# mindazhao/PWStableNet

Measured on AMD Instinct MI355X. Metric: stabilized frames/sec at 256x256 (netG fp32 + grid_sample), whole job, higher is better.
Workload: dtype f32

## Files before the change

### pwstablenet_amd/csrc/conv_mfma.hip

```cpp
#include "conv_common.h"

namespace pws {

template <int KS_, int STRIDE_, int PAD_, int SUBPIX_, int TH_, int TW_, int TN_, int CK_, int WM_, int WN_, int MT_,
          int NT_, bool NCHW_ = false>
struct ConvCfg {
    static constexpr int KS = KS_, STRIDE = STRIDE_, PAD = PAD_, TH = TH_, TW = TW_, TN = TN_, CK = CK_;
    static constexpr int SUBPIX = SUBPIX_;
    static constexpr bool CONVT = SUBPIX_ != 0, NCHW = NCHW_;
    static constexpr int WM = WM_, WN = WN_, MT = MT_, NT = NT_;
    static constexpr int THREADS = 64 * WM * WN;
    static constexpr int BM = TH * TW * TN, BN = 32 * NT * WN;
    static_assert(BM == 32 * MT * WM, "tile pixels must equal the M extent of the wave grid");
    static constexpr int IH = (TH - 1) * STRIDE + KS, IW = (TW - 1) * STRIDE + KS;
    static constexpr int PIX = TN * IH * IW;
    static constexpr int CKP = CK + 1;
    static constexpr int TAPS = KS * KS;
    static constexpr int LDS_IN = (PIX * CKP + 3) / 4 * 4;
    static constexpr int LDS_W = TAPS * CK * BN;
    static constexpr int LDS_BYTES = (LDS_IN + LDS_W) * 4;
    static constexpr int C4 = CK / 4;
    static constexpr int ITEMS_IN = (PIX * C4 + THREADS - 1) / THREADS;
    static constexpr int ITEMS_W = (TAPS * CK * (BN / 4) + THREADS - 1) / THREADS;
    static constexpr int ITEMS_NCHW = (PIX * CK + THREADS - 1) / THREADS;
// ... 47 lines not shown
        const int item = tid + it * C::THREADS;
        const int row = item / (C::BN / 4), q = item % (C::BN / 4);
        const int tap = row / C::CK, c = row % C::CK;
        const bool ok = item < C::TAPS * C::CK * (C::BN / 4) && (co0 + q * 4) < p.cout;
        w_off[it] = ok ? (tap * p.cin_pad + c) * p.cout + co0 + q * 4 : 0;
        w_mask |= ok ? (1u << it) : 0u;
    }
    const float *w_cls = p.w + (size_t)cls * C::TAPS * p.cin_pad * p.cout;
    float4 r_in[C::NCHW ? 1 : C::ITEMS_IN];
    float4 r_w[C::ITEMS_W];
    float r_nchw[C::NCHW ? C::ITEMS_NCHW : 1];

    auto load_chunk = [&](int s, int c0, int wrow) {
        if constexpr (C::NCHW) {
            const int Creal = p.src_c[0];
            const size_t sstride = p.src_ld[0] ? (size_t)p.src_ld[0] : (size_t)Creal * p.H * p.W;
#pragma unroll
            for (int it = 0; it < C::ITEMS_NCHW; ++it) {
                const int item = tid + it * C::THREADS;
                const int c = item / C::PIX, pix = item % C::PIX;
                const int lx = pix % C::IW, ly = (pix / C::IW) % C::IH, tn = pix / (C::IW * C::IH);
                const int n = n0 + tn, iy = iy0 + ly, ix = ix0 + lx;
                const bool ok = item < C::PIX * C::CK && (c0 + c) < Creal && n < p.N && iy >= 0 && iy < p.H && ix >= 0 &&
                                ix < p.W;
                const size_t off = ok ? (size_t)n * sstride + ((size_t)(c0 + c) * p.H + iy) * p.W + ix : 0;
                const float v = p.src_ptr[0][off];
                r_nchw[it] = ok ? v : 0.f;
            }
        } else {
            const float *sp = p.src_ptr[s] + c0;
            const size_t ld = p.src_ld[s];
#pragma unroll
            for (int it = 0; it < C::ITEMS_IN; ++it)
                r_in[it] = *reinterpret_cast<const float4 *>(sp + (size_t)g_pix[it] * ld + g_c4[it]);
        }
        const float *wp = w_cls + (size_t)wrow * p.cout;
#pragma unroll
        for (int it = 0; it < C::ITEMS_W; ++it) r_w[it] = *reinterpret_cast<const float4 *>(wp + w_off[it]);
    };
    auto store_chunk = [&]() {
        if constexpr (C::NCHW) {
#pragma unroll
            for (int it = 0; it < C::ITEMS_NCHW; ++it) {
                const int item = tid + it * C::THREADS;
                const int c = item / C::PIX, pix = item % C::PIX;
                if (item < C::PIX * C::CK) lds_in[pix * C::CKP + c] = r_nchw[it];
            }
        } else {
#pragma unroll
            for (int it = 0; it < C::ITEMS_IN; ++it) {
                if (l_off[it] >= 0) {
                    const bool ok = (ok_mask >> it) & 1u;
                    float *d = lds_in + l_off[it];
                    d[0] = ok ? r_in[it].x : 0.f, d[1] = ok ? r_in[it].y : 0.f, d[2] = ok ? r_in[it].z : 0.f,
                    d[3] = ok ? r_in[it].w : 0.f;
                }
            }
        }
#pragma unroll
        for (int it = 0; it < C::ITEMS_W; ++it) {
            const int item = tid + it * C::THREADS;
            if (item < C::TAPS * C::CK * (C::BN / 4)) {
                const bool ok = (w_mask >> it) & 1u;
                *reinterpret_cast<float4 *>(lds_w + item * 4) =
                    ok ? r_w[it] : make_float4(0.f, 0.f, 0.f, 0.f);
            }
        }
    };

    f32x16 acc[C::MT][C::NT];
#pragma unroll
    for (int mt = 0; mt < C::MT; ++mt)
#pragma unroll
        for (int nt = 0; nt < C::NT; ++nt)
#pragma unroll
            for (int r = 0; r < 16; ++r) acc[mt][nt][r] = 0.f;

    int a_base[C::MT];
#pragma unroll
    for (int mt = 0; mt < C::MT; ++mt) {
        const int m = (wm * C::MT + mt) * 32 + l31;
        const int tx = m % C::TW, ty = (m / C::TW) % C::TH, tn = m / (C::TW * C::TH);
        a_base[mt] = ((tn * C::IH + ty * C::STRIDE) * C::IW + tx * C::STRIDE) * C::CKP + hi;
    }
    const int b_base = hi * C::BN + wn * C::NT * 32 + l31;

    int total_chunks = 0;
    if constexpr (C::NCHW) {
        total_chunks = p.cin_pad / C::CK;
    } else {
        for (int s = 0; s < p.nsrc; ++s) total_chunks += p.src_c[s] / C::CK;
    }
    const int ch_begin = split * p.chunks_per_split;
    const int ch_end = min(total_chunks, ch_begin + p.chunks_per_split);
    int s = 0, c0 = ch_begin * C::CK, wrow = ch_begin * C::CK;
    if constexpr (!C::NCHW) {
        while (s < p.nsrc - 1 && c0 >= p.src_c[s]) c0 -= p.src_c[s], ++s;
    }
    if (ch_begin < ch_end) load_chunk(s, c0, wrow);
    for (int ch = ch_begin; ch < ch_end; ++ch) {
        __syncthreads();
        store_chunk();
        __syncthreads();
        c0 += C::CK, wrow += C::CK;
        if (!C::NCHW && c0 >= p.src_c[s]) ++s, c0 = 0;
        if (ch + 1 < ch_end) load_chunk(s, c0, wrow);

#pragma unroll
        for (int tap = 0; tap < C::TAPS; ++tap) {
            if (C::SUBPIX == 2 && ((!py && tap / C::KS) || (!px && tap % C::KS))) continue;
            const int toff = ((tap / C::KS) * C::IW + (tap % C::KS)) * C::CKP;
#pragma unroll
            for (int kk = 0; kk < C::CK / 2; ++kk) {
                float a[C::MT], b[C::NT];
#pragma unroll
                for (int mt = 0; mt < C::MT; ++mt) a[mt] = lds_in[a_base[mt] + toff + 2 * kk];
#pragma unroll
                for (int nt = 0; nt < C::NT; ++nt) b[nt] = lds_w[b_base + (tap * C::CK + 2 * kk) * C::BN + nt * 32];
#pragma unroll
                for (int mt = 0; mt < C::MT; ++mt)
#pragma unroll
                    for (int nt = 0; nt < C::NT; ++nt)
                        acc[mt][nt] = __builtin_amdgcn_mfma_f32_32x32x2f32(a[mt], b[nt], acc[mt][nt], 0, 0, 0);
            }
        }
    }

    const bool partial = p.ksplit > 1;
    float *part = p.out + (size_t)split * p.split_stride;
#pragma unroll
    for (int nt = 0; nt < C::NT; ++nt) {
        const int co = co0 + (wn * C::NT + nt) * 32 + l31;
        const bool co_ok = co < p.cout;
#pragma unroll
        for (int mt = 0; mt < C::MT; ++mt) {
#pragma unroll
            for (int r = 0; r < 16; ++r) {
                const int m = (wm * C::MT + mt) * 32 + (r & 3) + 8 * (r >> 2) + 4 * hi;
                const int tx = m % C::TW, ty = (m / C::TW) % C::TH, tn = m / (C::TW * C::TH);
                const int n = n0 + tn, y = y0 + ty, x = x0 + tx;
                const int oy = C::CONVT ? 2 * y + py : y, ox = C::CONVT ? 2 * x + px : x;
                if (co_ok && n < p.N && y < p.LH && x < p.LW && oy < p.OH && ox < p.OW) {
                    const size_t pix = (size_t)(n * p.OH + oy) * p.OW + ox;
                    if (partial)
                        part[pix * p.cout + co] = acc[mt][nt][r];
                    else
                        epi_store(p, pix, co, acc[mt][nt][r]);
                }
            }
        }
    }
}

__global__ void __launch_bounds__(256) splitk_reduce_kernel(const ConvKParams p, const float *__restrict__ partial,
                                                            size_t total4) {
    const size_t i = (size_t)blockIdx.x * 256 + threadIdx.x;
    if (i >= total4) return;
    float4 a = reinterpret_cast<const float4 *>(partial)[i];
    for (int s = 1; s < p.ksplit; ++s) {
        const float4 b = reinterpret_cast<const float4 *>(partial + (size_t)s * p.split_stride)[i];
        a.x += b.x, a.y += b.y, a.z += b.z, a.w += b.w;
    }
    const size_t pix = (i * 4) / p.cout;
    const int co = (int)((i * 4) % p.cout);
    if (p.io_bf16) {
        epi_store_pair16(p, pix, co, a.x, a.y), epi_store_pair16(p, pix, co + 2, a.z, a.w);
        return;
    }
    epi_store(p, pix, co, a.x), epi_store(p, pix, co + 1, a.y), epi_store(p, pix, co + 2, a.z), epi_store(p, pix, co + 3, a.w);
}

int launch_splitk_reduce(const ConvKParams &kp, const float *partial, size_t total4, hipStream_t st) {
    hipLaunchKernelGGL(splitk_reduce_kernel, dim3((unsigned)((total4 + 255) / 256)), dim3(256), 0, st, kp, partial, total4);
    return check_launch("splitk_reduce_kernel");
}

template <class C>
static int run_cfg(const ConvKParams &kp, const ConvChoice &c, hipStream_t st) { return launch_planned<&conv_mfma_kernel<C>>(kp, c, st, "conv_mfma_kernel"); }

template <class C, int KID>
static constexpr TileChoice choice() {
    return TileChoice{C::TH, C::TW, C::TN, C::CK, C::BN, KID, {{C::THREADS, C::LDS_BYTES}, {C::THREADS, C::LDS_BYTES}}, &run_cfg<C>};
}

using K3S1_T256 = ConvCfg<3, 1, 1, 0, 16, 16, 1, 16, 4, 1, 2, 2>;
using K3S1_T128 = ConvCfg<3, 1, 1, 0, 8, 16, 1, 16, 4, 1, 1, 2>;
using K3S1_T64 = ConvCfg<3, 1, 1, 0, 8, 8, 1, 16, 2, 2, 1, 1>;
using K3S1_T64N4 = ConvCfg<3, 1, 1, 0, 4, 4, 4, 16, 2, 2, 1, 1>;
using K3S1_T64N16 = ConvCfg<3, 1, 1, 0, 2, 2, 16, 16, 2, 2, 1, 1>;
using K3S2_T256 = ConvCfg<3, 2, 1, 0, 16, 16, 1, 8, 4, 1, 2, 2>;
using K3S2_T128 = ConvCfg<3, 2, 1, 0, 8, 16, 1, 16, 4, 1, 1, 2>;
using K3S2_T64 = ConvCfg<3, 2, 1, 0, 8, 8, 1, 16, 2, 2, 1, 1>;
using K3S2_T64N4 = ConvCfg<3, 2, 1, 0, 4, 4, 4, 16, 2, 2, 1, 1>;
using K3S2_T64N16 = ConvCfg<3, 2, 1, 0, 2, 2, 16, 16, 2, 2, 1, 1>;
using K5S1_T256 = ConvCfg<5, 1, 2, 0, 16, 16, 1, 8, 4, 1, 2, 2>;
using K5S1_T256_NCHW = ConvCfg<5, 1, 2, 0, 16, 16, 1, 8, 4, 1, 2, 2, true>;
using CT4_T256 = ConvCfg<2, 1, 0, 1, 16, 16, 1, 16, 4, 1, 2, 2>;
using CT4_T128 = ConvCfg<2, 1, 0, 1, 8, 16, 1, 16, 4, 1, 1, 2>;
using CT4_T64 = ConvCfg<2, 1, 0, 1, 8, 8, 1, 16, 2, 2, 1, 1>;
using CT4_T64N4 = ConvCfg<2, 1, 0, 1, 4, 4, 4, 16, 2, 2, 1, 1>;
using CT4_T64N16 = ConvCfg<2, 1, 0, 1, 2, 2, 16, 16, 2, 2, 1, 1>;

using K4S2_T256 = ConvCfg<4, 2, 1, 0, 16, 16, 1, 8, 4, 1, 2, 2>;
using K4S2_T128 = ConvCfg<4, 2, 1, 0, 8, 16, 1, 8, 4, 1, 1, 2>;
using K4S2_T64 = ConvCfg<4, 2, 1, 0, 8, 8, 1, 8, 2, 2, 1, 1>;
using K4S2_T64N4 = ConvCfg<4, 2, 1, 0, 4, 4, 4, 8, 2, 2, 1, 1>;
using K4S2_T64N16 = ConvCfg<4, 2, 1, 0, 2, 2, 16, 8, 2, 2, 1, 1>;
using SP3_T256 = ConvCfg<2, 1, 0, 2, 16, 16, 1, 16, 4, 1, 2, 2>;
using SP3_T128 = ConvCfg<2, 1, 0, 2, 8, 16, 1, 16, 4, 1, 1, 2>;
using SP3_T64 = ConvCfg<2, 1, 0, 2, 8, 8, 1, 16, 2, 2, 1, 1>;
using SP3_T64N4 = ConvCfg<2, 1, 0, 2, 4, 4, 4, 16, 2, 2, 1, 1>;
using SP3_T64N16 = ConvCfg<2, 1, 0, 2, 2, 2, 16, 16, 2, 2, 1, 1>;

static const TileChoice kK3S1[] = {choice<K3S1_T256, KID_CONV_K3S1_BIG>(), choice<K3S1_T128, KID_CONV_K3S1_BIG>(),
                                   choice<K3S1_T64, KID_CONV_K3S1_SMALL>(), choice<K3S1_T64N4, KID_CONV_K3S1_SMALL>(),
                                   choice<K3S1_T64N16, KID_CONV_K3S1_SMALL>()};
static const TileChoice kK3S2[] = {choice<K3S2_T256, KID_CONV_K3S2_BIG>(), choice<K3S2_T128, KID_CONV_K3S2_BIG>(),
                                   choice<K3S2_T64, KID_CONV_K3S2_SMALL>(), choice<K3S2_T64N4, KID_CONV_K3S2_SMALL>(),
                                   choice<K3S2_T64N16, KID_CONV_K3S2_SMALL>()};
static const TileChoice kCT4[] = {choice<CT4_T256, KID_CONVT4_BIG>(), choice<CT4_T128, KID_CONVT4_BIG>(),
                                  choice<CT4_T64, KID_CONVT4_SMALL>(), choice<CT4_T64N4, KID_CONVT4_SMALL>(),
                                  choice<CT4_T64N16, KID_CONVT4_SMALL>()};
static const TileChoice kK4S2[] = {choice<K4S2_T256, KID_DGRAD_K4S2>(), choice<K4S2_T128, KID_DGRAD_K4S2>(),
                                   choice<K4S2_T64, KID_DGRAD_K4S2>(), choice<K4S2_T64N4, KID_DGRAD_K4S2>(),
                                   choice<K4S2_T64N16, KID_DGRAD_K4S2>()};
static const TileChoice kSP3[] = {choice<SP3_T256, KID_DGRAD_SP3>(), choice<SP3_T128, KID_DGRAD_SP3>(),
                                  choice<SP3_T64, KID_DGRAD_SP3>(), choice<SP3_T64N4, KID_DGRAD_SP3>(),
                                  choice<SP3_T64N16, KID_DGRAD_SP3>()};
static const TileChoice kK5[] = {choice<K5S1_T256, KID_CONV_K5S1>()};
static const TileChoice kK5N[] = {choice<K5S1_T256_NCHW, KID_CONV_K5S1>()};

bool conv_mfma(int kind, bool dgrad, bool nchw, ConvKParams &kp, int cin_total, float *final_out, float *ws, size_t ws_floats, const ProfInfo &pi,
               const ConvCtx &cx, int *status) {
    const bool s1 = kind == PWS_CONV_K3S1 || kind == PWS_CONVT_K3S1, k5 = kind == PWS_CONV_K5S1;
    const TileChoice *cands = s1 ? kK3S1 : k5 ? (nchw ? kK5N : kK5) : kind == PWS_CONV_K3S2 ? (dgrad ? kSP3 : kK3S2) : (dgrad ? kK4S2 : kCT4);
    const int ncand = k5 ? 1 : 5;
    ConvChoice c;
    const TileChoice *t = plan_tiles(cands, ncand, kp, cin_total, final_out, ws, ws_floats, kFillBlocks, 0, &c);
    return conv_accept(cx, c, pi, status, [&] { return run_tiles(*t, c, kp, final_out, ws, cx.stream); });
}

}
```

### pwstablenet_amd/csrc/head.hip

```cpp
#include <type_traits>

#include "common.h"

namespace pws {

__device__ __forceinline__ float lrelu(float v) { return v > 0.f ? v : 0.2f * v; }

constexpr int TH_NB = 8;

__global__ void __launch_bounds__(64) theta_hidden_kernel(const float *__restrict__ x, int n, int k1, int hidden, int kchunk,
                                                          const float *__restrict__ w_flat, float *__restrict__ partial) {
    extern __shared__ float sx[];
    const int lane = threadIdx.x;
    const int j = blockIdx.x * 64 + lane;
    const int slice = blockIdx.y;
    const int k0 = slice * kchunk, kn = min(kchunk, k1 - k0);
    for (int n0 = blockIdx.z * TH_NB; n0 < n; n0 += gridDim.z * TH_NB) {
        const int nb = min(TH_NB, n - n0);
        __syncthreads();
        for (int i = lane; i < nb * kn; i += 64) sx[(i / kn) * kchunk + i % kn] = x[(size_t)(n0 + i / kn) * k1 + k0 + i % kn];
        __syncthreads();
        float acc[TH_NB];
#pragma unroll
        for (int s = 0; s < TH_NB; ++s) acc[s] = 0.f;
        if (j < hidden) {
            for (int kb = 0; kb < kn; kb += 8) {
                float wv[8];
#pragma unroll
                for (int u = 0; u < 8; ++u) wv[u] = w_flat[(size_t)(k0 + (kb + u < kn ? kb + u : kb)) * hidden + j];
#pragma unroll
                for (int u = 0; u < 8; ++u) {
                    if (kb + u < kn) {
#pragma unroll
                        for (int s = 0; s < TH_NB; ++s) acc[s] = fmaf(s < nb ? sx[s * kchunk + kb + u] : 0.f, wv[u], acc[s]);
                    }
                }
            }
#pragma unroll
            for (int s = 0; s < TH_NB; ++s)
                if (s < nb) partial[((size_t)slice * n + n0 + s) * hidden + j] = acc[s];
        }
    }
}

__global__ void __launch_bounds__(256) theta_final_kernel(const float *__restrict__ partial, int nslices, int n, int hidden,
                                                          const float *__restrict__ b_flat, const float *__restrict__ w_lin,
                                                          const float *__restrict__ b_lin, float *__restrict__ theta,
                                                          float *__restrict__ h_saved) {
    extern __shared__ float sh[];
    const int s = blockIdx.x, tid = threadIdx.x;
    for (int j = tid; j < hidden; j += 256) {
        float acc = b_flat ? b_flat[j] : 0.f;
        for (int sl = 0; sl < nslices; ++sl) acc += partial[((size_t)sl * n + s) * hidden + j];
        sh[j] = lrelu(acc);
        if (h_saved) h_saved[(size_t)s * hidden + j] = sh[j];
    }
    __syncthreads();
    const int wv = tid >> 6, lane = tid & 63;
    for (int o = wv; o < 6; o += 4) {
        float acc = 0.f;
        for (int j = lane; j < hidden; j += 64) acc = fmaf(sh[j], w_lin[(size_t)j * 6 + o], acc);
#pragma unroll
        for (int off = 32; off > 0; off >>= 1) acc += __shfl_down(acc, off, 64);
        if (lane == 0) theta[(size_t)s * 6 + o] = lrelu(acc + (b_lin ? b_lin[o] : 0.f));
    }
}

constexpr int FH_T = 16, FH_I = FH_T + 2, FH_CH = 16, FH_LDP = FH_CH + 4;

template <bool IO16>
__global__ void __launch_bounds__(256) field_head_kernel(const float *__restrict__ x, int ld, int N, int H, int W, int C,
                                                         const float *__restrict__ w_out, const float *__restrict__ b_out,
                                                         const float *__restrict__ theta, int ac, float *__restrict__ resid,
                                                         float *__restrict__ grid, int tiles_x, int tiles_y, unsigned ntiles, int raw) {
    __shared__ float s_in[FH_I * FH_I * FH_LDP];
    const int tid = threadIdx.x;
    const unsigned tile = xcd_remap(blockIdx.x, ntiles);
    const int tx_i = tile % tiles_x, ty_i = (tile / tiles_x) % tiles_y, n = tile / (tiles_x * tiles_y);
    const int x0 = tx_i * FH_T, y0 = ty_i * FH_T;
    const int tx = tid & 15, ty = tid >> 4;
    const int ch = C < FH_CH ? C : FH_CH;
    const int c4n = ch / 4;
    float acc0 = b_out ? b_out[0] : 0.f, acc1 = b_out ? b_out[1] : 0.f;
    constexpr int NITEM = (FH_I * FH_I * (FH_CH / 4) + 255) / 256;
    float4 pre[NITEM];
    auto fetch = [&](int c0) {
#pragma unroll
        for (int it = 0; it < NITEM; ++it) {
            const int item = tid + it * 256;
            const int pix = item / c4n, c4 = item % c4n;
            const int iy = y0 - 1 + pix / FH_I, ix = x0 - 1 + pix % FH_I;
            const bool ok = item < FH_I * FH_I * c4n && iy >= 0 && iy < H && ix >= 0 && ix < W;
            const float4 v = ld4<IO16>(x, ok ? ((size_t)(n * H + iy) * W + ix) * ld + c0 + c4 * 4 : 0);
            pre[it] = ok ? v : make_float4(0.f, 0.f, 0.f, 0.f);
        }
    };
    fetch(0);
    for (int c0 = 0; c0 < C; c0 += ch) {
        __syncthreads();
#pragma unroll
        for (int it = 0; it < NITEM; ++it) {
            const int item = tid + it * 256;
            if (item < FH_I * FH_I * c4n) *reinterpret_cast<float4 *>(s_in + (item / c4n) * FH_LDP + (item % c4n) * 4) = pre[it];
        }
        __syncthreads();
        if (c0 + ch < C) fetch(c0 + ch);
#pragma unroll
        for (int tap = 0; tap < 9; ++tap) {
            const float *ip = s_in + ((ty + tap / 3) * FH_I + tx + tap % 3) * FH_LDP;
            const float *wp = w_out + ((size_t)tap * C + c0) * 2;
            for (int c4 = 0; c4 < c4n; ++c4) {
                const float4 v = *reinterpret_cast<const float4 *>(ip + c4 * 4);
                const float *wq = wp + c4 * 8;
                acc0 = fmaf(v.x, wq[0], acc0), acc1 = fmaf(v.x, wq[1], acc1);
                acc0 = fmaf(v.y, wq[2], acc0), acc1 = fmaf(v.y, wq[3], acc1);
                acc0 = fmaf(v.z, wq[4], acc0), acc1 = fmaf(v.z, wq[5], acc1);
                acc0 = fmaf(v.w, wq[6], acc0), acc1 = fmaf(v.w, wq[7], acc1);
            }
        }
    }
    const int y = y0 + ty, xq = x0 + tx;
    if (y < H && xq < W && raw) {
        *reinterpret_cast<float2 *>(resid + (((size_t)n * H + y) * W + xq) * 2) = make_float2(acc0, acc1);
    } else if (y < H && xq < W) {
        const float r0 = tanhf(tanhf(acc0)), r1 = tanhf(tanhf(acc1));
        const size_t p = ((size_t)n * H + y) * W + xq;
        if (resid) *reinterpret_cast<float2 *>(resid + p * 2) = make_float2(r0, r1);
        if (grid) {
            float a0 = 0.f, a1 = 0.f;
            if (theta) {
                const float *t = theta + (size_t)n * 6;
                const float bx = ac ? (W > 1 ? (2.f * xq) / (float)(W - 1) - 1.f : 0.f) : (2.f * xq + 1.f) / (float)W - 1.f;
                const float by = ac ? (H > 1 ? (2.f * y) / (float)(H - 1) - 1.f : 0.f) : (2.f * y + 1.f) / (float)H - 1.f;
                a0 = t[0] * bx + t[1] * by + t[2];
                a1 = t[3] * bx + t[4] * by + t[5];
            }
            *reinterpret_cast<float2 *>(grid + p * 2) = make_float2(r0 + a0, r1 + a1);
        }
    }
}


__global__ void __launch_bounds__(256) field_head16_mfma_kernel(const __bf16 *__restrict__ x, int ld, int N, int H, int W,
                                                                const float *__restrict__ w_out, const float *__restrict__ b_out,
                                                                const float *__restrict__ theta, int ac, float *__restrict__ resid,
                                                                float *__restrict__ grid, int tiles_x, int tiles_y, unsigned ntiles, int raw) {
    constexpr int C = 64, NPIX = FH_I * FH_I, YP = 18;
    __shared__ float ys[NPIX * YP];
    typedef float f32x16 __attribute__((ext_vector_type(16)));
    const int tid = threadIdx.x, lane = tid & 63, wv = tid >> 6, l31 = lane & 31, hi = lane >> 5;
    bf16x8 bh[4], bl[4], bl2[4];
    {
        const int tap = l31 >> 1, o = l31 & 1;
#pragma unroll
        for (int ks = 0; ks < 4; ++ks)
#pragma unroll
            for (int i = 0; i < 8; ++i) {
                const float w = l31 < 18 ? w_out[((size_t)tap * C + ks * 16 + hi * 8 + i) * 2 + o] : 0.f;
                const __bf16 h = (__bf16)w;
                const float r1 = w - (float)h;
                const __bf16 m = (__bf16)r1;
                bh[ks][i] = h, bl[ks][i] = m, bl2[ks][i] = (__bf16)(r1 - (float)m);
            }
    }
    constexpr int MT = (NPIX + 31) / 32;
    constexpr int MTW = (MT + 3) / 4;
    bf16x8 a[MTW][4];
    auto load_tile = [&](unsigned t) {
        const unsigned tile = xcd_remap(t, ntiles);
        const int tx_i = tile % tiles_x, ty_i = (tile / tiles_x) % tiles_y, n = tile / (tiles_x * tiles_y);
        const int x0 = tx_i * FH_T, y0 = ty_i * FH_T;
#pragma unroll
        for (int i = 0; i < MTW; ++i) {
            const int q = (wv + 4 * i) * 32 + l31;
            const int iy = y0 - 1 + q / FH_I, ix = x0 - 1 + q % FH_I;
            const bool ok = q < NPIX && iy >= 0 && iy < H && ix >= 0 && ix < W;
            const __bf16 *px = x + (ok ? ((size_t)(n * H + iy) * W + ix) * ld + hi * 8 : 0);
#pragma unroll
            for (int ks = 0; ks < 4; ++ks) {
                const u32x4 v = *reinterpret_cast<const u32x4 *>(px + ks * 16);
                a[i][ks] = __builtin_bit_cast(bf16x8, ok ? v : (u32x4){0u, 0u, 0u, 0u});
            }
        }
    };
    unsigned t = blockIdx.x;
    if (t >= ntiles) return;
    load_tile(t);
    const float bias0 = b_out ? b_out[0] : 0.f, bias1 = b_out ? b_out[1] : 0.f;
    for (;;) {
        const unsigned tile = xcd_remap(t, ntiles);
        const int tx_i = tile % tiles_x, ty_i = (tile / tiles_x) % tiles_y, n = tile / (tiles_x * tiles_y);
        const int x0 = tx_i * FH_T, y0 = ty_i * FH_T;
#pragma unroll
        for (int i = 0; i < MTW; ++i) {
            const int mt = wv + 4 * i;
            if (mt >= MT) break;
            f32x16 acc;
#pragma unroll
            for (int r = 0; r < 16; ++r) acc[r] = 0.f;
#pragma unroll
            for (int ks = 0; ks < 4; ++ks) {
                acc = __builtin_amdgcn_mfma_f32_32x32x16_bf16(a[i][ks], bh[ks], acc, 0, 0, 0);
                acc = __builtin_amdgcn_mfma_f32_32x32x16_bf16(a[i][ks], bl[ks], acc, 0, 0, 0);
                acc = __builtin_amdgcn_mfma_f32_32x32x16_bf16(a[i][ks], bl2[ks], acc, 0, 0, 0);
            }
            if (l31 < 18) {
#pragma unroll
                for (int r = 0; r < 16; ++r) {
                    const int qq = mt * 32 + (r & 3) + 8 * (r >> 2) + 4 * hi;
                    if (qq < NPIX) ys[qq * YP + l31] = acc[r];
                }
            }
        }
        const unsigned tn = t + gridDim.x;
// ... 158 lines not shown
        }
        __syncthreads();
#pragma unroll
        for (int h2 = 0; h2 < 2; ++h2) {
            const int idx = tid + h2 * 256;
            const int ty = idx >> 5, tx = idx & 31;
            float acc0 = bias0, acc1 = bias1;
#pragma unroll
            for (int tap = 0; tap < 9; ++tap) {
                const float2 v = *reinterpret_cast<const float2 *>(ysr + (h2 * 8 * F2_IW + (tap / 3) * F2_IW + tap % 3) * F2_YP + tap * 2);
                acc0 += v.x, acc1 += v.y;
            }
            const int y = T.y0 + ty, xq = T.x0 + tx;
            if (y < H && xq < W && raw) {
                *reinterpret_cast<float2 *>(resid + (((size_t)T.n * H + y) * W + xq) * 2) = make_float2(acc0, acc1);
            } else if (y < H && xq < W) {
                const float r0 = tanhf(tanhf(acc0)), r1 = tanhf(tanhf(acc1));
                const size_t pp = ((size_t)T.n * H + y) * W + xq;
                if (resid) *reinterpret_cast<float2 *>(resid + pp * 2) = make_float2(r0, r1);
                if (grid) {
                    float a0 = 0.f, a1 = 0.f;
                    if (theta) {
                        const float *th = theta + (size_t)T.n * 6;
                        const float bx = (ac && W <= 1) ? 0.f : (float)(2 * xq + 1 - ac) / (float)(W - ac) - 1.f;
                        const float by = (ac && H <= 1) ? 0.f : (float)(2 * y + 1 - ac) / (float)(H - ac) - 1.f;
                        a0 = th[0] * bx + th[1] * by + th[2];
                        a1 = th[3] * bx + th[4] * by + th[5];
                    }
                    *reinterpret_cast<float2 *>(grid + pp * 2) = make_float2(r0 + a0, r1 + a1);
                }
            }
        }
        __syncthreads();
    };
    auto advance = [&]() {
        T = TN, t = tn, tn += gridDim.x;
        more = tn < ntiles;
        if (more) TN = decode(tn);
    };
    for (;;) {
        do_tile(std::integral_constant<int, 0>{});
        if (!more) break;
        advance();
        do_tile(std::integral_constant<int, F2_BPW % NSET>{});
        if (!more) break;
        advance();
        if constexpr (NSET == 3) {
            do_tile(std::integral_constant<int, (2 * F2_BPW) % NSET>{});
            if (!more) break;
            advance();
        }
    }
}

__global__ void __launch_bounds__(256) field_head32_mfma_kernel(const float *__restrict__ x, int ld, int N, int H, int W,
                                                                const float *__restrict__ w_out, const float *__restrict__ b_out,
                                                                const float *__restrict__ theta, int ac, float *__restrict__ resid,
                                                                float *__restrict__ grid, int tiles_x, int tiles_y, unsigned ntiles, int raw) {
    constexpr int C = 64, NPIX = FH_I * FH_I, YP = 18;
    __shared__ float ys[NPIX * YP];
    typedef float f32x16 __attribute__((ext_vector_type(16)));
    const int tid = threadIdx.x, lane = tid & 63, wv = tid >> 6, l31 = lane & 31, hi = lane >> 5;
    float bw[32];
    {
        const int tap = l31 >> 1, o = l31 & 1;
#pragma unroll
        for (int j = 0; j < 32; ++j) bw[j] = l31 < 18 ? w_out[((size_t)tap * C + hi * 32 + j) * 2 + o] : 0.f;
    }
    constexpr int MT = (NPIX + 31) / 32, MTW = (MT + 3) / 4;
    f32x4 a[MTW][8];
    auto load_tile = [&](unsigned t) {
        const unsigned tile = xcd_remap(t, ntiles);
        const int tx_i = tile % tiles_x, ty_i = (tile / tiles_x) % tiles_y, n = tile / (tiles_x * tiles_y);
        const int x0 = tx_i * FH_T, y0 = ty_i * FH_T;
#pragma unroll
        for (int i = 0; i < MTW; ++i) {
            const int q = (wv + 4 * i) * 32 + l31;
            const int iy = y0 - 1 + q / FH_I, ix = x0 - 1 + q % FH_I;
            const bool ok = q < NPIX && iy >= 0 && iy < H && ix >= 0 && ix < W;
            const float *px = x + (ok ? ((size_t)(n * H + iy) * W + ix) * ld + hi * 32 : 0);
#pragma unroll
            for (int k4 = 0; k4 < 8; ++k4) {
                const f32x4 v = *reinterpret_cast<const f32x4 *>(px + k4 * 4);
                a[i][k4] = ok ? v : (f32x4){0.f, 0.f, 0.f, 0.f};
            }
        }
    };
    unsigned t = blockIdx.x;
    if (t >= ntiles) return;
    load_tile(t);
    const float bias0 = b_out ? b_out[0] : 0.f, bias1 = b_out ? b_out[1] : 0.f;
    for (;;) {
        const unsigned tile = xcd_remap(t, ntiles);
        const int tx_i = tile % tiles_x, ty_i = (tile / tiles_x) % tiles_y, n = tile / (tiles_x * tiles_y);
        const int x0 = tx_i * FH_T, y0 = ty_i * FH_T;
#pragma unroll
        for (int i = 0; i < MTW; ++i) {
            const int mt = wv + 4 * i;
            if (mt >= MT) break;
            f32x16 acc;
#pragma unroll
            for (int r = 0; r < 16; ++r) acc[r] = 0.f;
#pragma unroll
            for (int j = 0; j < 32; ++j) acc = __builtin_amdgcn_mfma_f32_32x32x2f32(a[i][j >> 2][j & 3], bw[j], acc, 0, 0, 0);
            if (l31 < 18) {
#pragma unroll
                for (int r = 0; r < 16; ++r) {
                    const int qq = mt * 32 + (r & 3) + 8 * (r >> 2) + 4 * hi;
                    if (qq < NPIX) ys[qq * YP + l31] = acc[r];
                }
            }
        }
        const unsigned tn = t + gridDim.x;
        const bool more = tn < ntiles;
        if (more) load_tile(tn);
        __syncthreads();
        const int tx = tid & 15, ty = tid >> 4;
        float acc0 = bias0, acc1 = bias1;
#pragma unroll
        for (int tap = 0; tap < 9; ++tap) {
            const float2 v = *reinterpret_cast<const float2 *>(ys + ((ty + tap / 3) * FH_I + tx + tap % 3) * YP + tap * 2);
            acc0 += v.x, acc1 += v.y;
        }
        const int y = y0 + ty, xq = x0 + tx;
        if (y < H && xq < W && raw) {
            *reinterpret_cast<float2 *>(resid + (((size_t)n * H + y) * W + xq) * 2) = make_float2(acc0, acc1);
        } else if (y < H && xq < W) {
            const float r0 = tanhf(tanhf(acc0)), r1 = tanhf(tanhf(acc1));
            const size_t p = ((size_t)n * H + y) * W + xq;
            if (resid) *reinterpret_cast<float2 *>(resid + p * 2) = make_float2(r0, r1);
            if (grid) {
                float a0 = 0.f, a1 = 0.f;
                if (theta) {
                    const float *th = theta + (size_t)n * 6;
                    const float bx = ac ? (W > 1 ? (2.f * xq) / (float)(W - 1) - 1.f : 0.f) : (2.f * xq + 1.f) / (float)W - 1.f;
                    const float by = ac ? (H > 1 ? (2.f * y) / (float)(H - 1) - 1.f : 0.f) : (2.f * y + 1.f) / (float)H - 1.f;
                    a0 = th[0] * bx + th[1] * by + th[2];
                    a1 = th[3] * bx + th[4] * by + th[5];
                }
                *reinterpret_cast<float2 *>(grid + p * 2) = make_float2(r0 + a0, r1 + a1);
            }
        }
        if (!more) break;
        __syncthreads();
        t = tn;
    }
}

__global__ void __launch_bounds__(256) theta_sum_kernel(const float *__restrict__ partial, int nslices, int n, int hidden,
                                                        const float *__restrict__ b_flat, float *__restrict__ z1) {
    const size_t e = (size_t)blockIdx.x * 256 + threadIdx.x;
    if (e >= (size_t)n * hidden) return;
    const int j = (int)(e % hidden);
    float acc = b_flat ? b_flat[j] : 0.f;
    for (int sl = 0; sl < nslices; ++sl) acc += partial[(size_t)sl * n * hidden + e];
    z1[e] = acc;
}
__global__ void __launch_bounds__(256) theta_z2_kernel(const float *__restrict__ h, int n, int hidden, const float *__restrict__ w_lin,
                                                       const float *__restrict__ b_lin, float *__restrict__ z2) {
    const int wave = (int)(((size_t)blockIdx.x * 256 + threadIdx.x) >> 6), lane = threadIdx.x & 63;
    if (wave >= n * 6) return;
    const int s = wave / 6, o = wave % 6;
    float acc = 0.f;
    for (int j = lane; j < hidden; j += 64) acc = fmaf(h[(size_t)s * hidden + j], w_lin[(size_t)j * 6 + o], acc);
#pragma unroll
    for (int off = 32; off > 0; off >>= 1) acc += __shfl_down(acc, off, 64);
    if (lane == 0) z2[(size_t)s * 6 + o] = acc + (b_lin ? b_lin[o] : 0.f);
}
__global__ void __launch_bounds__(256) field_bn_finish_kernel(const float *__restrict__ yhat, const float *__restrict__ theta, int H, int W,
                                                              size_t total, int ac, float *__restrict__ resid, float *__restrict__ grid) {
    const size_t p = (size_t)blockIdx.x * 256 + threadIdx.x;
    if (p >= total) return;
    const float2 v = *reinterpret_cast<const float2 *>(yhat + p * 2);
    const float r0 = tanhf(tanhf(v.x)), r1 = tanhf(tanhf(v.y));
    if (resid) *reinterpret_cast<float2 *>(resid + p * 2) = make_float2(r0, r1);
    if (grid) {
        const int xq = (int)(p % W), y = (int)((p / W) % H);
        const size_t n = p / ((size_t)W * H);
        float a0 = 0.f, a1 = 0.f;
        if (theta) {
            const float *t = theta + n * 6;
            const float bx = ac ? (W > 1 ? (2.f * xq) / (float)(W - 1) - 1.f : 0.f) : (2.f * xq + 1.f) / (float)W - 1.f;
            const float by = ac ? (H > 1 ? (2.f * y) / (float)(H - 1) - 1.f : 0.f) : (2.f * y + 1.f) / (float)H - 1.f;
            a0 = t[0] * bx + t[1] * by + t[2], a1 = t[3] * bx + t[4] * by + t[5];
        }
        *reinterpret_cast<float2 *>(grid + p * 2) = make_float2(r0 + a0, r1 + a1);
    }
}

}

using namespace pws;

static int theta_slices(int k1) {
    int kchunk = 64;
    return (k1 + kchunk - 1) / kchunk;
}

namespace pws {
int theta_z1(const float *x, int n, int c, int hidden, const float *w_flat, const float *b_flat, float *ws, float *z1, hipStream_t st) {
    const int k1 = 4 * c, kchunk = 64, nslices = theta_slices(k1);
    hipLaunchKernelGGL(theta_hidden_kernel, dim3((hidden + 63) / 64, nslices, (unsigned)((n + TH_NB - 1) / TH_NB)), dim3(64), sizeof(float) * TH_NB * kchunk, st, x, n, k1, hidden,
                       kchunk, w_flat, ws);
    const size_t e = (size_t)n * hidden;
    hipLaunchKernelGGL(theta_sum_kernel, dim3((unsigned)((e + 255) / 256)), dim3(256), 0, st, ws, nslices, n, hidden, b_flat, z1);
    return check_launch("theta_z1 kernels");
}
int theta_z2(const float *h, int n, int hidden, const float *w_lin, const float *b_lin, float *z2, hipStream_t st) {
    const size_t waves = (size_t)n * 6;
    hipLaunchKernelGGL(theta_z2_kernel, dim3((unsigned)((waves * 64 + 255) / 256)), dim3(256), 0, st, h, n, hidden, w_lin, b_lin, z2);
    return check_launch("theta_z2_kernel");
}
int field_head_raw(const float *x, int ld, int n, int h, int w, int c, const float *w_out, const float *b_out, float *z, hipStream_t st) {
    const int tiles_x = (w + FH_T - 1) / FH_T, tiles_y = (h + FH_T - 1) / FH_T;
    const unsigned ntiles = (unsigned)tiles_x * tiles_y * n;
    hipLaunchKernelGGL(field_head_kernel<false>, dim3(ntiles), dim3(256), 0, st, x, ld, n, h, w, c, w_out, b_out, (const float *)nullptr, 0, z,
                       (float *)nullptr, tiles_x, tiles_y, ntiles, 1);
    return check_launch("field_head_kernel<raw>");
}
int field_bn_finish(const float *yhat, const float *theta, int n, int h, int w, int ac, float *resid, float *grid, hipStream_t st) {
    const size_t total = (size_t)n * h * w;
    hipLaunchKernelGGL(field_bn_finish_kernel, dim3((unsigned)((total + 255) / 256)), dim3(256), 0, st, yhat, theta, h, w, total, ac, resid,
                       grid);
    return check_launch("field_bn_finish_kernel");
}
}

extern "C" size_t pws_theta_head_ws_floats(int n, int c, int hidden) {
    if (n <= 0 || c <= 0 || hidden <= 0) return 0;
    return (size_t)theta_slices(4 * c) * n * hidden;
}

extern "C" int pws_theta_head_fwd(const float *x, int n, int c, int hidden, const float *w_flat, const float *b_flat,
                                  const float *w_lin, const float *b_lin, float *ws, float *theta, pws_stream_t stream) {
    return pws_theta_head_fwd_save(x, n, c, hidden, w_flat, b_flat, w_lin, b_lin, ws, theta, nullptr, stream);
}

extern "C" int pws_theta_head_fwd_save(const float *x, int n, int c, int hidden, const float *w_flat, const float *b_flat,
                                       const float *w_lin, const float *b_lin, float *ws, float *theta, float *h_saved,
                                       pws_stream_t stream) {
    PWS_REQUIRE(n >= 0 && c > 0 && hidden > 0, "pws_theta_head_fwd: bad shape");
    if (n == 0) return PWS_OK;
    PWS_REQUIRE(x && w_flat && w_lin && theta && ws, "pws_theta_head_fwd: NULL pointer (ws needs pws_theta_head_ws_floats())");
    const int k1 = 4 * c, kchunk = 64, nslices = theta_slices(k1);
    PWS_REQUIRE(hidden * sizeof(float) <= 64 * 1024, "pws_theta_head_fwd: hidden = %d exceeds 64 KB of LDS", hidden);
    ProfScope prof(KID_THETA_HEAD, 2.0 * n * ((double)k1 * hidden + 6.0 * hidden), 4.0 * ((double)k1 * hidden + n * k1),
                   as_stream(stream));
    hipLaunchKernelGGL(theta_hidden_kernel, dim3((hidden + 63) / 64, nslices, (unsigned)((n + TH_NB - 1) / TH_NB)), dim3(64), sizeof(float) * TH_NB * kchunk,
                       as_stream(stream), x, n, k1, hidden, kchunk, w_flat, ws);
    hipLaunchKernelGGL(theta_final_kernel, dim3(n), dim3(256), sizeof(float) * hidden, as_stream(stream), ws, nslices, n, hidden,
                       b_flat, w_lin, b_lin, theta, h_saved);
    return check_launch("theta_head kernels");
}

extern "C" int pws_field_head_fwd(const float *x, int ld, int n, int h, int w, int c, const float *w_out, const float *b_out,
                                  const float *theta, int align_corners, float *resid, float *grid, pws_stream_t stream) {
    return pws_field_head_fwd_s(x, ld, n, h, w, c, w_out, b_out, theta, align_corners, resid, grid, PWS_STORE_FP32, stream);
}

extern "C" int pws_field_head_fwd_s(const float *x, int ld, int n, int h, int w, int c, const float *w_out, const float *b_out,
                                    const float *theta, int align_corners, float *resid, float *grid, int store,
                                    pws_stream_t stream) {
    PWS_REQUIRE(n >= 0 && h > 0 && w > 0 && c > 0, "pws_field_head_fwd: bad shape");
    if (n == 0) return PWS_OK;
    PWS_REQUIRE(x && w_out && (resid || grid), "pws_field_head_fwd: NULL pointer");
    const int ch = c < FH_CH ? c : FH_CH;
    PWS_REQUIRE(c % 4 == 0 && c % ch == 0 && ld % 4 == 0 && ld >= c && (reinterpret_cast<size_t>(x) & 15) == 0,
                "pws_field_head_fwd: c=%d must be a multiple of 4 (and of 16 when > 16), ld %% 4 == 0, x 16-B aligned", c);
    const int tiles_x = (w + FH_T - 1) / FH_T, tiles_y = (h + FH_T - 1) / FH_T;
    const unsigned ntiles = (unsigned)tiles_x * tiles_y * n;
    ProfScope prof(KID_FIELD_HEAD, 2.0 * n * h * w * 18.0 * c,
                   (double)n * h * w * (4.0 * c + (resid ? 8.0 : 0.0) + (grid ? 8.0 : 0.0)), as_stream(stream));
    const int ncu = device_cus();
    unsigned pgrid = ntiles;
    if (!exp_is(EXP_HEAD_ONE_TILE) && ntiles > (unsigned)(ncu * 3)) {
        const unsigned k = (ntiles + (unsigned)(ncu * 3) - 1) / (unsigned)(ncu * 3);
        pgrid = ((ntiles + k - 1) / k + kXcds - 1) / kXcds * kXcds;
    }
    const bool v2_16 = store == PWS_STORE_BF16 && ld % 8 == 0, v2_32 = store != PWS_STORE_BF16;
    if (c == 64 && (v2_16 || v2_32) && !exp_is(EXP_HEAD_VALU) && !exp_is(EXP_HEAD_V1) && w >= F2_TW && h >= F2_TH && (long long)h * w * ld * 4 < (1ll << 30)) {
        const int tx2 = (w + F2_TW - 1) / F2_TW, ty2 = (h + F2_TH - 1) / F2_TH;
        const unsigned nt2 = (unsigned)tx2 * ty2 * n;
        unsigned pg2 = nt2;
        if (!exp_is(EXP_HEAD_ONE_TILE) && nt2 > (unsigned)(ncu * 3)) {
            const unsigned k = (nt2 + (unsigned)(ncu * 3) - 1) / (unsigned)(ncu * 3);
            pg2 = ((nt2 + k - 1) / k + kXcds - 1) / kXcds * kXcds;
        }
        if (v2_16)
            hipLaunchKernelGGL((field_head_v2_kernel<false, 3>), dim3(pg2), dim3(256), 0, as_stream(stream), x, ld, n, h, w, w_out, b_out, theta, align_corners, resid,
                               grid, tx2, ty2, nt2, 0);
        else
            hipLaunchKernelGGL((field_head_v2_kernel<true, 2>), dim3(pg2), dim3(256), 0, as_stream(stream), x, ld, n, h, w, w_out, b_out, theta, align_corners, resid,
                               grid, tx2, ty2, nt2, 0);
    } else if (store == PWS_STORE_BF16 && c == 64 && ld % 8 == 0 && !exp_is(EXP_HEAD_VALU))
        hipLaunchKernelGGL(field_head16_mfma_kernel, dim3(pgrid), dim3(256), 0, as_stream(stream), reinterpret_cast<const __bf16 *>(x), ld, n, h, w,
                           w_out, b_out, theta, align_corners, resid, grid, tiles_x, tiles_y, ntiles, 0);
    else if (store == PWS_STORE_BF16)
        hipLaunchKernelGGL(field_head_kernel<true>, dim3(ntiles), dim3(256), 0, as_stream(stream), x, ld, n, h, w, c, w_out, b_out,
                           theta, align_corners, resid, grid, tiles_x, tiles_y, ntiles, 0);
    else if (c == 64 && !exp_is(EXP_HEAD_VALU))
        hipLaunchKernelGGL(field_head32_mfma_kernel, dim3(pgrid), dim3(256), 0, as_stream(stream), x, ld, n, h, w, w_out, b_out, theta, align_corners,
                           resid, grid, tiles_x, tiles_y, ntiles, 0);
    else
        hipLaunchKernelGGL(field_head_kernel<false>, dim3(ntiles), dim3(256), 0, as_stream(stream), x, ld, n, h, w, c, w_out, b_out,
                           theta, align_corners, resid, grid, tiles_x, tiles_y, ntiles, 0);
    return check_launch("field_head_kernel");
}
```

Before: 2031.

## Batch loads in split-K reduce and restructure theta head kernels for ILP

Result: no change. 2049, median of 6 (+0.9%).

```diff
diff --git a/pwstablenet_amd/csrc/conv_mfma.hip b/pwstablenet_amd/csrc/conv_mfma.hip
--- a/pwstablenet_amd/csrc/conv_mfma.hip
+++ b/pwstablenet_amd/csrc/conv_mfma.hip
@@ -223,22 +223,57 @@
     }
 }
 
+constexpr int SK_B = 8;
+
 __global__ void __launch_bounds__(256) splitk_reduce_kernel(const ConvKParams p, const float *__restrict__ partial,
                                                             size_t total4) {
     const size_t i = (size_t)blockIdx.x * 256 + threadIdx.x;
     if (i >= total4) return;
-    float4 a = reinterpret_cast<const float4 *>(partial)[i];
-    for (int s = 1; s < p.ksplit; ++s) {
-        const float4 b = reinterpret_cast<const float4 *>(partial + (size_t)s * p.split_stride)[i];
-        a.x += b.x, a.y += b.y, a.z += b.z, a.w += b.w;
-    }
-    const size_t pix = (i * 4) / p.cout;
-    const int co = (int)((i * 4) % p.cout);
+    size_t pix;
+    int co;
+    if (total4 <= 0x3fffffffu) {
+        const unsigned e = (unsigned)i * 4u;
+        pix = e / (unsigned)p.cout, co = (int)(e % (unsigned)p.cout);
+    } else {
+        pix = (i * 4) / p.cout, co = (int)((i * 4) % p.cout);
+    }
+    const float4 *src = reinterpret_cast<const float4 *>(partial) + i;
+    const bool plain = p.ndst == 0, has_bias = plain && p.bias != nullptr;
+    const float *bp = has_bias ? p.bias + co : reinterpret_cast<const float *>(src);
+    const float4 bl = make_float4(bp[0], bp[1], bp[2], bp[3]);
+    const float4 bias = make_float4(has_bias ? bl.x : 0.f, has_bias ? bl.y : 0.f, has_bias ? bl.z : 0.f, has_bias ? bl.w : 0.f);
+    const size_t stride4 = p.split_stride / 4;
+    const int last = p.ksplit - 1;
+    float4 a = make_float4(0.f, 0.f, 0.f, 0.f);
+    for (int s0 = 0; s0 <= last; s0 += SK_B) {
+        float4 b[SK_B];
+#pragma unroll
+        for (int u = 0; u < SK_B; ++u) b[u] = src[(size_t)min(s0 + u, last) * stride4];
+#pragma unroll
+        for (int u = 0; u < SK_B; ++u) {
+            const float4 t = make_float4(a.x + b[u].x, a.y + b[u].y, a.z + b[u].z, a.w + b[u].w);
+            const bool first = u == 0 && s0 == 0;
+            const bool on = s0 + u <= last;
+            a.x = first ? b[u].x : (on ? t.x : a.x), a.y = first ? b[u].y : (on ? t.y : a.y);
+            a.z = first ? b[u].z : (on ? t.z : a.z), a.w = first ? b[u].w : (on ? t.w : a.w);
+        }
+    }
+    const float4 v = make_float4(a.x + bias.x, a.y + bias.y, a.z + bias.z, a.w + bias.w);
     if (p.io_bf16) {
-        epi_store_pair16(p, pix, co, a.x, a.y), epi_store_pair16(p, pix, co + 2, a.z, a.w);
+        if (plain) {
+            unsigned *d = reinterpret_cast<unsigned *>(reinterpret_cast<__bf16 *>(p.out) + pix * p.out_ld + co);
+            d[0] = cvt_pk_bf16(act_apply(v.x, p.act), act_apply(v.y, p.act)), d[1] = cvt_pk_bf16(act_apply(v.z, p.act), act_apply(v.w, p.act));
+        } else {
+            epi_store_pair16(p, pix, co, a.x, a.y), epi_store_pair16(p, pix, co + 2, a.z, a.w);
+        }
         return;
     }
-    epi_store(p, pix, co, a.x), epi_store(p, pix, co + 1, a.y), epi_store(p, pix, co + 2, a.z), epi_store(p, pix, co + 3, a.w);
+    if (plain) {
+        float *d = p.out + pix * p.out_ld + co;
+        d[0] = act_apply(v.x, p.act), d[1] = act_apply(v.y, p.act), d[2] = act_apply(v.z, p.act), d[3] = act_apply(v.w, p.act);
+    } else {
+        epi_store(p, pix, co, a.x), epi_store(p, pix, co + 1, a.y), epi_store(p, pix, co + 2, a.z), epi_store(p, pix, co + 3, a.w);
+    }
 }
 
 int launch_splitk_reduce(const ConvKParams &kp, const float *partial, size_t total4, hipStream_t st) {
diff --git a/pwstablenet_amd/csrc/head.hip b/pwstablenet_amd/csrc/head.hip
--- a/pwstablenet_amd/csrc/head.hip
+++ b/pwstablenet_amd/csrc/head.hip
@@ -7,40 +7,70 @@
 __device__ __forceinline__ float lrelu(float v) { return v > 0.f ? v : 0.2f * v; }
 
 constexpr int TH_NB = 8;
-
-__global__ void __launch_bounds__(64) theta_hidden_kernel(const float *__restrict__ x, int n, int k1, int hidden, int kchunk,
+constexpr int TH_KC = 64;
+
+__global__ void __launch_bounds__(64) theta_hidden_kernel(const float *__restrict__ x, int n, int k1, int hidden,
                                                           const float *__restrict__ w_flat, float *__restrict__ partial) {
-    extern __shared__ float sx[];
+    __shared__ __attribute__((aligned(16))) float sx[TH_NB * TH_KC];
     const int lane = threadIdx.x;
-    const int j = blockIdx.x * 64 + lane;
+    const int j = blockIdx.x * 64 + lane, jc = min(j, hidden - 1);
     const int slice = blockIdx.y;
-    const int k0 = slice * kchunk, kn = min(kchunk, k1 - k0);
+    const int k0 = slice * TH_KC, kn = min(TH_KC, k1 - k0);
+    float *out = partial + (size_t)slice * n * hidden + j;
+    if (kn < TH_KC) {
+        for (int n0 = blockIdx.z * TH_NB; n0 < n; n0 += gridDim.z * TH_NB) {
+            for (int s = n0; s < min(n, n0 + TH_NB); ++s) {
+                float acc = 0.f;
+                for (int k = 0; k < kn; ++k) acc = fmaf(x[(size_t)s * k1 + k0 + k], w_flat[(size_t)(k0 + k) * hidden + jc], acc);
+                if (j < hidden) out[(size_t)s * hidden] = acc;
+            }
+        }
+        return;
+    }
+    float wv[TH_KC];
+#pragma unroll
+    for (int k = 0; k < TH_KC; ++k) wv[k] = w_flat[(size_t)(k0 + k) * hidden + jc];
     for (int n0 = blockIdx.z * TH_NB; n0 < n; n0 += gridDim.z * TH_NB) {
-        const int nb = min(TH_NB, n - n0);
-        __syncthreads();
-        for (int i = lane; i < nb * kn; i += 64) sx[(i / kn) * kchunk + i % kn] = x[(size_t)(n0 + i / kn) * k1 + k0 + i % kn];
-        __syncthreads();
-        float acc[TH_NB];
-#pragma unroll
-        for (int s = 0; s < TH_NB; ++s) acc[s] = 0.f;
+        float xr[TH_NB];
+#pragma unroll
+        for (int s = 0; s < TH_NB; ++s) xr[s] = x[(size_t)min(n0 + s, n - 1) * k1 + k0 + lane];
+        __syncthreads();
+#pragma unroll
+        for (int s = 0; s < TH_NB; ++s) sx[s * TH_KC + lane] = xr[s];
+        __syncthreads();
         if (j < hidden) {
-            for (int kb = 0; kb < kn; kb += 8) {
-                float wv[8];
-#pragma unroll
-                for (int u = 0; u < 8; ++u) wv[u] = w_flat[(size_t)(k0 + (kb + u < kn ? kb + u : kb)) * hidden + j];
-#pragma unroll
-                for (int u = 0; u < 8; ++u) {
-                    if (kb + u < kn) {
-#pragma unroll
-                        for (int s = 0; s < TH_NB; ++s) acc[s] = fmaf(s < nb ? sx[s * kchunk + kb + u] : 0.f, wv[u], acc[s]);
-                    }
-                }
-            }
-#pragma unroll
-            for (int s = 0; s < TH_NB; ++s)
-                if (s < nb) partial[((size_t)slice * n + n0 + s) * hidden + j] = acc[s];
-        }
-    }
+            float acc[TH_NB];
+#pragma unroll
+            for (int s = 0; s < TH_NB; ++s) acc[s] = 0.f;
+#pragma unroll
+            for (int kb = 0; kb < TH_KC; kb += 4) {
+#pragma unroll
+                for (int s = 0; s < TH_NB; ++s) {
+                    const float4 xv = *reinterpret_cast<const float4 *>(sx + s * TH_KC + kb);
+                    acc[s] = fmaf(xv.x, wv[kb], acc[s]), acc[s] = fmaf(xv.y, wv[kb + 1], acc[s]);
+                    acc[s] = fmaf(xv.z, wv[kb + 2], acc[s]), acc[s] = fmaf(xv.w, wv[kb + 3], acc[s]);
+                }
+            }
+#pragma unroll
+            for (int s = 0; s < TH_NB; ++s) out[(size_t)min(n0 + s, n - 1) * hidden] = acc[s];
+        }
+    }
+}
+
+constexpr int TH_SB = 8;
+template <class F>
+__device__ __forceinline__ float add_in_order(float acc, int count, F &&v) {
+    for (int s0 = 0; s0 < count; s0 += TH_SB) {
+        float b[TH_SB];
+#pragma unroll
+        for (int u = 0; u < TH_SB; ++u) b[u] = v(min(s0 + u, count - 1));
+#pragma unroll
+        for (int u = 0; u < TH_SB; ++u) {
+            const float t = acc + b[u];
+            acc = s0 + u < count ? t : acc;
+        }
+    }
+    return acc;
 }
 
 __global__ void __launch_bounds__(256) theta_final_kernel(const float *__restrict__ partial, int nslices, int n, int hidden,
@@ -50,8 +80,8 @@
     extern __shared__ float sh[];
     const int s = blockIdx.x, tid = threadIdx.x;
     for (int j = tid; j < hidden; j += 256) {
-        float acc = b_flat ? b_flat[j] : 0.f;
-        for (int sl = 0; sl < nslices; ++sl) acc += partial[((size_t)sl * n + s) * hidden + j];
+        const float *pj = partial + (size_t)s * hidden + j;
+        const float acc = add_in_order(b_flat ? b_flat[j] : 0.f, nslices, [&](int sl) { return pj[(size_t)sl * n * hidden]; });
         sh[j] = lrelu(acc);
         if (h_saved) h_saved[(size_t)s * hidden + j] = sh[j];
     }
@@ -59,7 +89,17 @@
     const int wv = tid >> 6, lane = tid & 63;
     for (int o = wv; o < 6; o += 4) {
         float acc = 0.f;
-        for (int j = lane; j < hidden; j += 64) acc = fmaf(sh[j], w_lin[(size_t)j * 6 + o], acc);
+        for (int j0 = lane; j0 < hidden; j0 += 8 * 64) {
+            float w[8];
+#pragma unroll
+            for (int u = 0; u < 8; ++u) w[u] = w_lin[(size_t)(j0 + u * 64 < hidden ? j0 + u * 64 : lane) * 6 + o];
+#pragma unroll
+            for (int u = 0; u < 8; ++u) {
+                const bool on = j0 + u * 64 < hidden;
+                const float t = fmaf(sh[on ? j0 + u * 64 : lane], w[u], acc);
+                acc = on ? t : acc;
+            }
+        }
 #pragma unroll
         for (int off = 32; off > 0; off >>= 1) acc += __shfl_down(acc, off, 64);
         if (lane == 0) theta[(size_t)s * 6 + o] = lrelu(acc + (b_lin ? b_lin[o] : 0.f));
@@ -524,9 +564,7 @@
     const size_t e = (size_t)blockIdx.x * 256 + threadIdx.x;
     if (e >= (size_t)n * hidden) return;
     const int j = (int)(e % hidden);
-    float acc = b_flat ? b_flat[j] : 0.f;
-    for (int sl = 0; sl < nslices; ++sl) acc += partial[(size_t)sl * n * hidden + e];
-    z1[e] = acc;
+    z1[e] = add_in_order(b_flat ? b_flat[j] : 0.f, nslices, [&](int sl) { return partial[(size_t)sl * n * hidden + e]; });
 }
 __global__ void __launch_bounds__(256) theta_z2_kernel(const float *__restrict__ h, int n, int hidden, const float *__restrict__ w_lin,
                                                        const float *__restrict__ b_lin, float *__restrict__ z2) {
@@ -564,16 +602,13 @@
 
 using namespace pws;
 
-static int theta_slices(int k1) {
-    int kchunk = 64;
-    return (k1 + kchunk - 1) / kchunk;
-}
+static int theta_slices(int k1) { return (k1 + TH_KC - 1) / TH_KC; }
 
 namespace pws {
 int theta_z1(const float *x, int n, int c, int hidden, const float *w_flat, const float *b_flat, float *ws, float *z1, hipStream_t st) {
-    const int k1 = 4 * c, kchunk = 64, nslices = theta_slices(k1);
-    hipLaunchKernelGGL(theta_hidden_kernel, dim3((hidden + 63) / 64, nslices, (unsigned)((n + TH_NB - 1) / TH_NB)), dim3(64), sizeof(float) * TH_NB * kchunk, st, x, n, k1, hidden,
-                       kchunk, w_flat, ws);
+    const int k1 = 4 * c, nslices = theta_slices(k1);
+    hipLaunchKernelGGL(theta_hidden_kernel, dim3((hidden + 63) / 64, nslices, (unsigned)((n + TH_NB - 1) / TH_NB)), dim3(64), 0, st, x, n, k1, hidden,
+                       w_flat, ws);
     const size_t e = (size_t)n * hidden;
     hipLaunchKernelGGL(theta_sum_kernel, dim3((unsigned)((e + 255) / 256)), dim3(256), 0, st, ws, nslices, n, hidden, b_flat, z1);
     return check_launch("theta_z1 kernels");
@@ -614,12 +649,12 @@
     PWS_REQUIRE(n >= 0 && c > 0 && hidden > 0, "pws_theta_head_fwd: bad shape");
     if (n == 0) return PWS_OK;
     PWS_REQUIRE(x && w_flat && w_lin && theta && ws, "pws_theta_head_fwd: NULL pointer (ws needs pws_theta_head_ws_floats())");
-    const int k1 = 4 * c, kchunk = 64, nslices = theta_slices(k1);
+    const int k1 = 4 * c, nslices = theta_slices(k1);
     PWS_REQUIRE(hidden * sizeof(float) <= 64 * 1024, "pws_theta_head_fwd: hidden = %d exceeds 64 KB of LDS", hidden);
     ProfScope prof(KID_THETA_HEAD, 2.0 * n * ((double)k1 * hidden + 6.0 * hidden), 4.0 * ((double)k1 * hidden + n * k1),
                    as_stream(stream));
-    hipLaunchKernelGGL(theta_hidden_kernel, dim3((hidden + 63) / 64, nslices, (unsigned)((n + TH_NB - 1) / TH_NB)), dim3(64), sizeof(float) * TH_NB * kchunk,
-                       as_stream(stream), x, n, k1, hidden, kchunk, w_flat, ws);
+    hipLaunchKernelGGL(theta_hidden_kernel, dim3((hidden + 63) / 64, nslices, (unsigned)((n + TH_NB - 1) / TH_NB)), dim3(64), 0,
+                       as_stream(stream), x, n, k1, hidden, w_flat, ws);
     hipLaunchKernelGGL(theta_final_kernel, dim3(n), dim3(256), sizeof(float) * hidden, as_stream(stream), ws, nslices, n, hidden,
                        b_flat, w_lin, b_lin, theta, h_saved);
     return check_launch("theta_head kernels");
```
